# MrTornado24/IDE-3D

Hardware: AMD Instinct MI355X
Metric: 512x512 RGB+seg frames/s @96 depth samples (whole job) (higher is better)
Workload: dtype f32 (3x3 convs + MLPs: fp32 operands as 3 bf16 pieces, 6 products, f32 accumulate); 1 GPU; BASELINE config 2: random-init ide3d-ffhq-64-512, G.mapping + G.synthesis (64 render -> 512, 96 samples, RGB + 19-class seg) + uint8 frames, batch 4 seeds per GPU; global_batch=4, parallelism=dp1, conv_arithmetic=bf16x6, conv_arithmetic_is_library_default=True

## Files before the change

### ide-3d_amd/csrc/raymarch.hip

```cpp
#include "common.h"
#include "triplane_tap.h"
#include "raymarch_ray.h"

namespace ide3d {

typedef float f32x4 __attribute__((ext_vector_type(4)));

template <int C, int HID>
struct RmCfg {
    static constexpr int CPL = C / 16;
    static constexpr int NF = C / 4;
    static constexpr int MT1 = HID / 16;
    static constexpr int MT2 = 2;
    static constexpr int A1 = MT1 * CPL * 64 * 4;
    static constexpr int A2 = MT2 * MT1 * 64 * 4;
    static constexpr int B0 = MT1 * 16;
    static constexpr int B1 = MT2 * 16;
    static constexpr int MLP = A1 + A2 + B0 + B1;
};

template <int HID>
__device__ __forceinline__ void stage_out_fp32(float* __restrict__ a2, const float* __restrict__ w1, int nout) {
    constexpr int MT1 = HID / 16;
    for (int i = threadIdx.x; i < 2 * MT1 * 64 * 4; i += blockDim.x) {
// ... 58 lines not shown
        split_pair3(v[2 * e], v[2 * e + 1], pk);
        out[0][e] = pk[0]; out[1][e] = pk[1]; out[2][e] = pk[2];
    }
}
__device__ __forceinline__ f32x4 mfma6(const u32x4 (&a)[3], const u32x4 (&b)[3], f32x4 acc) {
#pragma unroll
    for (int sum = 2; sum >= 0; --sum)
#pragma unroll
        for (int qa = 0; qa <= sum; ++qa)
            acc = __builtin_amdgcn_mfma_f32_16x16x32_bf16(__builtin_bit_cast(bf16x8, a[qa]), __builtin_bit_cast(bf16x8, b[sum - qa]), acc, 0, 0, 0);
    return acc;
}

template <int C, int HID>
__device__ __forceinline__ void stage_split_layer1(u32x4* __restrict__ a1, const float* __restrict__ w0) {
    using K = RmSplit<C, HID>;
    for (int i = threadIdx.x; i < K::MT1 * 64; i += blockDim.x) {
        const int lane = i & 63, mt = i >> 6, g = lane >> 4, row = 16 * mt + (lane & 15);
        float v[8];
#pragma unroll
        for (int k = 0; k < 8; ++k) v[k] = w0[row * C + 16 * (k / 4) + 4 * g + k % 4];
        u32x4 pc[3];
        split8(v, pc);
#pragma unroll
        for (int q = 0; q < 3; ++q) a1[(mt * 3 + q) * 64 + lane] = pc[q];
    }
}
template <int HID>
__device__ __forceinline__ void stage_split_biases(float* __restrict__ sb, const float* __restrict__ b0, const float* __restrict__ b1, int nout) {
    for (int i = threadIdx.x; i < HID; i += blockDim.x) sb[i] = b0[i];
    for (int i = threadIdx.x; i < 32; i += blockDim.x) sb[HID + i] = (i < nout) ? b1[i] : 0.f;
}

template <int C, int HID>
__device__ void stage_mlp_split(unsigned char* __restrict__ sm, const float* __restrict__ w0, const float* __restrict__ b0,
                                const float* __restrict__ w1, const float* __restrict__ b1, int nout) {
    using K = RmSplit<C, HID>;
    u32x4* a1 = reinterpret_cast<u32x4*>(sm);
    u32x4* a2 = a1 + K::A1;
    stage_split_layer1<C, HID>(a1, w0);
    for (int i = threadIdx.x; i < 2 * K::KH * 64; i += blockDim.x) {
        const int lane = i & 63, kh = (i >> 6) % K::KH, m2 = i / (64 * K::KH), g = lane >> 4, row = 16 * m2 + (lane & 15);
        float v[8];
#pragma unroll
        for (int k = 0; k < 8; ++k) v[k] = (row < nout) ? w1[row * HID + 16 * (2 * kh + k / 4) + 4 * g + k % 4] : 0.f;
        u32x4 pc[3];
        split8(v, pc);
#pragma unroll
        for (int q = 0; q < 3; ++q) a2[((m2 * K::KH + kh) * 3 + q) * 64 + lane] = pc[q];
    }
    stage_split_biases<HID>(reinterpret_cast<float*>(a2 + K::A2), b0, b1, nout);
}

template <int C, int HID, int A2U = RmSplit<C, HID>::A2>
__device__ __forceinline__ void mlp_hidden_split(const unsigned char* __restrict__ sm, const float (&f)[C / 4], f32x4 (&h)[HID / 16]) {
    using K = RmSplit<C, HID>;
    const int lane = lane_id(), g = lane >> 4;
    const u32x4* a1 = reinterpret_cast<const u32x4*>(sm);
    const f32x4* sb0 = reinterpret_cast<const f32x4*>(sm + (K::A1 + A2U) * 16);
    u32x4 fb[3];
    split8(f, fb);
#pragma unroll
    for (int mt = 0; mt < K::MT1; ++mt) {
        const u32x4 a[3] = {a1[(mt * 3 + 0) * 64 + lane], a1[(mt * 3 + 1) * 64 + lane], a1[(mt * 3 + 2) * 64 + lane]};
        h[mt] = mfma6(a, fb, sb0[mt * 4 + g]);
    }
#pragma unroll
    for (int mt = 0; mt < K::MT1; ++mt)
#pragma unroll
        for (int r = 0; r < 4; ++r) h[mt][r] = softplus_fast(h[mt][r]);
}

template <int C, int HID>
__device__ __forceinline__ void mlp_tile_split(const unsigned char* __restrict__ sm, const float (&f)[C / 4], f32x4 (&out)[2]) {
    using K = RmSplit<C, HID>;
    const int lane = lane_id(), g = lane >> 4;
    const u32x4* a2 = reinterpret_cast<const u32x4*>(sm) + K::A1;
    const f32x4* sb1 = reinterpret_cast<const f32x4*>(sm + (K::A1 + K::A2) * 16) + K::MT1 * 4;
    f32x4 h[K::MT1];
    mlp_hidden_split<C, HID>(sm, f, h);
    u32x4 hb[K::KH][3];
#pragma unroll
    for (int kh = 0; kh < K::KH; ++kh) {
        const float v[8] = {h[2 * kh][0], h[2 * kh][1], h[2 * kh][2], h[2 * kh][3], h[2 * kh + 1][0], h[2 * kh + 1][1], h[2 * kh + 1][2], h[2 * kh + 1][3]};
        split8(v, hb[kh]);
    }
#pragma unroll
    for (int m2 = 0; m2 < 2; ++m2) {
        f32x4 acc = sb1[m2 * 4 + g];
#pragma unroll
        for (int kh = 0; kh < K::KH; ++kh) {
            const int o = ((m2 * K::KH + kh) * 3) * 64 + lane;
            const u32x4 a[3] = {a2[o], a2[o + 64], a2[o + 128]};
            acc = mfma6(a, hb[kh], acc);
        }
        out[m2] = acc;
    }
}

template <int HID>
__device__ __forceinline__ float sigma_row0(const float* __restrict__ s_row, const f32x4 (&h)[HID / 16]) {
    const int g = lane_id() >> 4;
    float acc = 0.f;
#pragma unroll
    for (int mt = 0; mt < HID / 16; ++mt) {
        const f32x4 w = *reinterpret_cast<const f32x4*>(s_row + 16 * mt + 4 * g);
#pragma unroll
        for (int r = 0; r < 4; ++r) acc += w[r] * h[mt][r];
    }
    acc += __shfl_xor(acc, 16);
    acc += __shfl_xor(acc, 32);
    return acc + s_row[HID];
}

template <int C, int HID>
__device__ __forceinline__ float mlp_sigma_split(const unsigned char* __restrict__ sm, const float* __restrict__ s_row, const float (&f)[C / 4]) {
    f32x4 h[HID / 16];
    mlp_hidden_split<C, HID>(sm, f, h);
    return sigma_row0<HID>(s_row, h);
}

__device__ __forceinline__ int gather_sample(int lane) { return lane >> 2; }
__device__ __forceinline__ int gather_block(int lane) { return lane & 3; }

template <int NF>
__device__ __forceinline__ void to_matrix_lanes(float (&f)[NF]) {
    const int lane = lane_id();
    const int src = (((lane & 15) << 2) | (lane >> 4)) << 2;
#pragma unroll
    for (int i = 0; i < NF; ++i) f[i] = __int_as_float(__builtin_amdgcn_ds_bpermute(src, __float_as_int(f[i])));
}

template <int C> struct TapBuf { float4 v[C / 16][3][4]; };

typedef const __attribute__((address_space(1))) char* GlobalBytes;
template <class T>
__device__ __forceinline__ GlobalBytes uniform_ptr(const T* p) {
    const unsigned long long v = reinterpret_cast<unsigned long long>(p);
    const unsigned lo = __builtin_amdgcn_readfirstlane((unsigned)v), hi = __builtin_amdgcn_readfirstlane((unsigned)(v >> 32));
    return reinterpret_cast<GlobalBytes>(((unsigned long long)hi << 32) | lo);
}

__device__ __forceinline__ float4 ld4_at(GlobalBytes base, unsigned byte_off, unsigned imm) {
    typedef float v4f __attribute__((ext_vector_type(4)));
    typedef const __attribute__((address_space(1))) v4f* GlobalF4;
    const v4f v = *reinterpret_cast<GlobalF4>(base + (size_t)byte_off + imm);
    return make_float4(v[0], v[1], v[2], v[3]);
}

template <int C>
__device__ __forceinline__ void issue_taps(GlobalBytes pbc, const TapAddr (&t)[3], int g, TapBuf<C>& b, unsigned lane_extra = 0) {
    constexpr int CPL = C / 16;
    const unsigned lane_b = 16u * (unsigned)g + lane_extra;
#pragma unroll
    for (int ci = 0; ci < CPL; ++ci) {
#pragma unroll
        for (int pl = 0; pl < 3; ++pl) {
            const unsigned imm = (unsigned)(pl * C + 16 * ci) * 4u;
            b.v[ci][pl][0] = ld4_at(pbc, (unsigned)t[pl].o00 * 4u + lane_b, imm); b.v[ci][pl][1] = ld4_at(pbc, (unsigned)t[pl].o01 * 4u + lane_b, imm);
            b.v[ci][pl][2] = ld4_at(pbc, (unsigned)t[pl].o10 * 4u + lane_b, imm); b.v[ci][pl][3] = ld4_at(pbc, (unsigned)t[pl].o11 * 4u + lane_b, imm);
        }
    }
}

template <int C>
__device__ __forceinline__ void blend_taps(TapBuf<C>& b, const TapAddr (&t)[3], float (&f)[C / 4]) {
    constexpr int CPL = C / 16;
#pragma unroll
    for (int ci = 0; ci < CPL; ++ci)
#pragma unroll
        for (int pl = 0; pl < 3; ++pl)
#pragma unroll
            for (int k = 0; k < 4; ++k) asm volatile("" : "+v"(b.v[ci][pl][k].x), "+v"(b.v[ci][pl][k].y), "+v"(b.v[ci][pl][k].z), "+v"(b.v[ci][pl][k].w));
#pragma unroll
    for (int ci = 0; ci < CPL; ++ci) {
        float4 a[3];
#pragma unroll
        for (int pl = 0; pl < 3; ++pl) {
            float4 acc = make_float4(0.f, 0.f, 0.f, 0.f);
            acc = f4_fma(b.v[ci][pl][0], t[pl].w00, acc);
            acc = f4_fma(b.v[ci][pl][1], t[pl].w01, acc);
            acc = f4_fma(b.v[ci][pl][2], t[pl].w10, acc);
            acc = f4_fma(b.v[ci][pl][3], t[pl].w11, acc);
            a[pl] = acc;
        }
        f[4 * ci + 0] = (a[0].x + a[1].x) + a[2].x;
        f[4 * ci + 1] = (a[0].y + a[1].y) + a[2].y;
        f[4 * ci + 2] = (a[0].z + a[1].z) + a[2].z;
        f[4 * ci + 3] = (a[0].w + a[1].w) + a[2].w;
    }
}

template <int C>
__device__ __forceinline__ void gather_features(const float* __restrict__ pb, const TapAddr (&t)[3], int g, float (&f)[C / 4]) {
    TapBuf<C> b;
    issue_taps<C>(uniform_ptr(pb), t, g, b);
    blend_taps<C>(b, t, f);
}

template <int C, int HID>
__device__ __forceinline__ void mlp_hidden(const float* __restrict__ s, const float (&f)[C / 4], f32x4 (&h)[HID / 16]) {
    using K = RmCfg<C, HID>;
    const int lane = lane_id();
    const f32x4* a1 = reinterpret_cast<const f32x4*>(s);
    const f32x4* sb0 = reinterpret_cast<const f32x4*>(s + K::A1 + K::A2);
    const int g = lane >> 4;
#pragma unroll
    for (int mt = 0; mt < K::MT1; ++mt) h[mt] = sb0[mt * 4 + g];
#pragma unroll
    for (int ci = 0; ci < K::CPL; ++ci) {
        f32x4 w[K::MT1];
#pragma unroll
        for (int mt = 0; mt < K::MT1; ++mt) w[mt] = a1[(mt * K::CPL + ci) * 64 + lane];
#pragma unroll
        for (int e = 0; e < 4; ++e)
#pragma unroll
            for (int mt = 0; mt < K::MT1; ++mt)
                h[mt] = __builtin_amdgcn_mfma_f32_16x16x4f32(w[mt][e], f[4 * ci + e], h[mt], 0, 0, 0);
    }
#pragma unroll
    for (int mt = 0; mt < K::MT1; ++mt)
#pragma unroll
        for (int r = 0; r < 4; ++r) h[mt][r] = softplus_fast(h[mt][r]);
}

template <int C, int HID>
__device__ __forceinline__ void mlp_tile(const float* __restrict__ s, const float (&f)[C / 4], f32x4 (&out)[2]) {
    using K = RmCfg<C, HID>;
    const int lane = lane_id();
    const f32x4* a2 = reinterpret_cast<const f32x4*>(s + K::A1);
    const f32x4* sb1 = reinterpret_cast<const f32x4*>(s + K::A1 + K::A2 + K::B0);
    const int g = lane >> 4;
    f32x4 h[K::MT1];
    mlp_hidden<C, HID>(s, f, h);
#pragma unroll
    for (int mt = 0; mt < 2; ++mt) out[mt] = sb1[mt * 4 + g];
#pragma unroll
    for (int tq = 0; tq < K::MT1; ++tq) {
        const f32x4 w0 = a2[(0 * K::MT1 + tq) * 64 + lane];
        const f32x4 w1 = a2[(1 * K::MT1 + tq) * 64 + lane];
#pragma unroll
        for (int e = 0; e < 4; ++e) {
            out[0] = __builtin_amdgcn_mfma_f32_16x16x4f32(w0[e], h[tq][e], out[0], 0, 0, 0);
            out[1] = __builtin_amdgcn_mfma_f32_16x16x4f32(w1[e], h[tq][e], out[1], 0, 0, 0);
        }
    }
}

template <int C, int HID>
__device__ __forceinline__ float mlp_sigma(const float* __restrict__ s, const float* __restrict__ s_row, const float (&f)[C / 4]) {
    f32x4 h[HID / 16];
    mlp_hidden<C, HID>(s, f, h);
    return sigma_row0<HID>(s_row, h);
}

__device__ __forceinline__ float seg16_excl_prod(float v, float& total) {
    const int j = lane_id() & 15;
    float incl = v;
#pragma unroll
    for (int off = 1; off < 16; off <<= 1) {
        const float o = __shfl_up(incl, off, 16);
        if (j >= off) incl *= o;
    }
    total = __shfl(incl, 15, 16);
    const float prev = __shfl_up(incl, 1, 16);
    return j == 0 ? 1.0f : prev;
}

template <int C, int HID, bool SPLIT> struct MlpBytes { static constexpr int value = RmCfg<C, HID>::MLP * 4; };
template <int C, int HID> struct MlpBytes<C, HID, true> { static constexpr int value = RmSplit<C, HID>::BYTES; };

template <int C, int HID, bool SPLIT>
__device__ __forceinline__ void stage_branch(unsigned char* sm, const float* w0, const float* b0, const float* w1, const float* b1, int nout) {
    if constexpr (SPLIT) stage_mlp_split<C, HID>(sm, w0, b0, w1, b1, nout);
    else stage_mlp<C, HID>(reinterpret_cast<float*>(sm), w0, b0, w1, b1, nout);
}
template <int C, int HID, bool SPLIT>
__device__ __forceinline__ void mlp_branch(const unsigned char* sm, const float (&f)[C / 4], f32x4 (&out)[2]) {
    if constexpr (SPLIT) mlp_tile_split<C, HID>(sm, f, out);
    else mlp_tile<C, HID>(reinterpret_cast<const float*>(sm), f, out);
}

template <int C, int HID, bool SPLIT> struct RmRender {
    using K = RmCfg<C, HID>;
    static constexpr int W2_OFF = K::A1 * 4, B1_OFF = (K::A1 + K::A2 + K::B0) * 4, BYTES = K::MLP * 4;
    static constexpr int ROW = HID + 4;
};
template <int C, int HID> struct RmRender<C, HID, true> {
    using K = RmSplit<C, HID>;
    static constexpr int W2 = 2 * K::MT1 * 64;
    static constexpr int W2_OFF = K::A1 * 16, B1_OFF = (K::A1 + W2) * 16 + HID * 4, BYTES = (K::A1 + W2) * 16 + K::BIAS * 4;
    static constexpr int ROW = HID + 4;
};

template <int C, int HID, bool SPLIT>
__device__ __forceinline__ void stage_render_branch(unsigned char* sm, const float* w0, const float* b0, const float* w1, const float* b1, int nout) {
    if constexpr (SPLIT) {
        using R = RmRender<C, HID, true>;
        stage_split_layer1<C, HID>(reinterpret_cast<u32x4*>(sm), w0);
        stage_out_fp32<HID>(reinterpret_cast<float*>(sm + R::W2_OFF), w1, nout);
        stage_split_biases<HID>(reinterpret_cast<float*>(sm + R::W2_OFF + R::W2 * 16), b0, b1, nout);
    } else {
        stage_mlp<C, HID>(reinterpret_cast<float*>(sm), w0, b0, w1, b1, nout);
    }
}
template <int C, int HID, bool SPLIT>
__device__ __forceinline__ void hidden_branch(const unsigned char* sm, const float (&f)[C / 4], f32x4 (&h)[HID / 16]) {
    if constexpr (SPLIT) mlp_hidden_split<C, HID, RmRender<C, HID, true>::W2>(sm, f, h);
    else mlp_hidden<C, HID>(reinterpret_cast<const float*>(sm), f, h);
}

template <int CTRL>
__device__ __forceinline__ float dpp_add(float v) {
    return v + __int_as_float(__builtin_amdgcn_update_dpp(0, __float_as_int(v), CTRL, 0xf, 0xf, false));
}
__device__ __forceinline__ float row16_sum(float v) {
    v = dpp_add<0xB1>(v); v = dpp_add<0x4E>(v); v = dpp_add<0x141>(v); v = dpp_add<0x140>(v);
    return v;
}

template <int C, int HID, bool SPLIT>
__device__ __forceinline__ void heads_per_ray(const unsigned char* sm, const float (&acc)[HID / 4], float wsum, float (&out)[2]) {
    using R = RmRender<C, HID, SPLIT>;
    constexpr int MT1 = HID / 16;
    const int lane = lane_id();
    const f32x4* w2 = reinterpret_cast<const f32x4*>(sm + R::W2_OFF);
    const float* sb1 = reinterpret_cast<const float*>(sm + R::B1_OFF);
#pragma unroll
    for (int m2 = 0; m2 < 2; ++m2) {
        float a = 0.f;
#pragma unroll
        for (int mt = 0; mt < MT1; ++mt) {
            const f32x4 w = w2[(m2 * MT1 + mt) * 64 + lane];
#pragma unroll
            for (int r = 0; r < 4; ++r) a = fmaf(w[r], acc[4 * mt + r], a);
        }
        a += __shfl_xor(a, 16);
        a += __shfl_xor(a, 32);
        out[m2] = fmaf(sb1[16 * m2 + (lane & 15)], wsum, a);
    }
}

template <bool SPLIT> struct RmWaves { static constexpr int value = SPLIT ? 8 : 4; };
template <bool SPLIT> __device__ __forceinline__ void rm_claim_half_simd() { if constexpr (SPLIT) asm volatile("" ::: "v255"); }

template <int C, int HID, bool SPLIT>
__global__ void __launch_bounds__(64 * RmWaves<SPLIT>::value, 2)
render_rays_kernel(ide3d_render_params p, int64_t rays_per_block) {
    using K = RmCfg<C, HID>;
    constexpr int NW = RmWaves<SPLIT>::value;
    rm_claim_half_simd<SPLIT>();
    extern __shared__ __attribute__((aligned(16))) float lds[];
    using R = RmRender<C, HID, SPLIT>;
    constexpr int NA = HID / 4;
    unsigned char* s_geo = reinterpret_cast<unsigned char*>(lds);
    unsigned char* s_tex = s_geo + R::BYTES;
    float* const s_row = reinterpret_cast<float*>(s_tex + R::BYTES);
    stage_render_branch<C, HID, SPLIT>(s_geo, p.geo_w0, p.geo_b0, p.geo_w1, p.geo_b1, 1 + p.seg_ch);
    stage_render_branch<C, HID, SPLIT>(s_tex, p.tex_w0, p.tex_b0, p.tex_w1, p.tex_b1, p.feat_ch);
    for (int i = threadIdx.x; i <= HID; i += blockDim.x) s_row[i] = (i < HID) ? p.geo_w1[i] : p.geo_b1[0];
    __syncthreads();

    const int lane = lane_id(), wid = __builtin_amdgcn_readfirstlane(threadIdx.x >> 6);
    const int g = lane >> 4, j = lane & 15, gl = gather_block(lane);
    const int64_t total_rays = (int64_t)p.n * p.rays_per_img;
    const int blk = xcd_remap(blockIdx.x, gridDim.x);
    const int64_t ray_begin = (int64_t)blk * rays_per_block;
    int64_t ray_end = ray_begin + rays_per_block;
    if (ray_end > total_rays) ray_end = total_rays;
    const int S = p.steps;
    const int nch = p.feat_ch + p.seg_ch;
    const int sH = (int)p.tex_stride[2], sW = (int)p.tex_stride[3];
    const float zstep = (S > 1) ? (p.z_lin[1] - p.z_lin[0]) : 0.f;

    auto tile_depth = [&](int64_t ray, int s0, float& zl, float& jl) {
        const int sl = min(s0 + gather_sample(lane), S - 1);
        zl = p.z_lin[sl];
        jl = p.jitter ? p.jitter[ray * S + sl] : 0.5f;
    };
    auto tile_taps = [&](int n, int r, float zl, float jl, TapAddr (&t)[3]) {
        float wx, wy, wz;
        ray_world_point(p, n, r, zl, jl, zstep, wx, wy, wz);
        t[0] = make_tap_addr(wx, wy, p.W, p.H, sH, sW);
        t[1] = make_tap_addr(wy, wz, p.W, p.H, sH, sW);
        t[2] = make_tap_addr(wx, wz, p.W, p.H, sH, sW);
    };

    int64_t ray = ray_begin + wid;
    int n = __builtin_amdgcn_readfirstlane((int)(ray / p.rays_per_img));
    int r = __builtin_amdgcn_readfirstlane((int)(ray - (int64_t)n * p.rays_per_img));
    int s0 = 0;
    bool have = ray < ray_end;
    TapAddr t[3];
    TapBuf<C> buf;
    if (have) {
        float zl, jl;
        tile_depth(ray, 0, zl, jl);
        tile_taps(n, r, zl, jl, t);
        issue_taps<C>(uniform_ptr(p.geo_planes + n * p.geo_stride[0]), t, gl, buf);
    }
    float acc_t[NA], acc_g[NA];
#pragma unroll
    for (int i = 0; i < NA; ++i) { acc_t[i] = 0.f; acc_g[i] = 0.f; }
    float carry = 1.0f, wsum = 0.f, dsum = 0.f;

    while (have) {
        int s0n = s0 + 16, nn = n, rn = r;
        int64_t rayn = ray;
        if (s0n >= S) {
            s0n = 0; rayn = ray + NW; rn = r + NW;
            while (rn >= p.rays_per_img) { rn -= (int)p.rays_per_img; ++nn; }
        }
        const bool haven = rayn < ray_end;
        const int64_t rayp = haven ? rayn : ray;
        const int np = haven ? nn : n, rp = haven ? rn : r, s0p = haven ? s0n : s0;
        const int s = s0 + j;
        const bool live = s < S;
        const int sc = live ? s : S - 1;
        float z = p.z_lin[sc];
        float znext = (sc + 1 < S) ? p.z_lin[sc + 1] : 0.f;
        if (p.jitter) {
            const float* jit = p.jitter + ray * S;
            z = __fadd_rn(z, __fmul_rn(__fsub_rn(jit[sc], 0.5f), zstep));
            if (sc + 1 < S) znext = __fadd_rn(znext, __fmul_rn(__fsub_rn(jit[sc + 1], 0.5f), zstep));
        }
        const float noise = p.sigma_noise ? p.sigma_noise[ray * S + sc] : 0.f;
        float zln, jln;
        tile_depth(rayp, s0p, zln, jln);

        float fg[K::NF], ft[K::NF];
        f32x4 hg[K::MT1], ht[K::MT1];
        blend_taps<C>(buf, t, fg);
        to_matrix_lanes(fg);
        issue_taps<C>(uniform_ptr(p.tex_planes + n * p.tex_stride[0]), t, gl, buf);
        hidden_branch<C, HID, SPLIT>(s_geo, fg, hg);

        float sigma = sigma_row0<HID>(s_row, hg);
        sigma += noise;
        const float dens = p.clamp_mode == 0 ? softplus_fast(sigma) : fmaxf(sigma, 0.f);
        float dnorm;
        {
            const float dx = p.rays_d_cam[r * 3 + 0], dy = p.rays_d_cam[r * 3 + 1], dz = p.rays_d_cam[r * 3 + 2];
            dnorm = sqrtf(dx * dx + dy * dy + dz * dz);
        }
        const float delta = (sc + 1 < S) ? (znext - z) * dnorm : 1e10f;
        const float alpha = live ? 1.0f - __expf(-delta * dens) : 0.f;
        const float fac = live ? (1.0f - alpha + 1e-10f) : 1.0f;
        float tot;
        const float excl = seg16_excl_prod(fac, tot);
        const float w = alpha * (carry * excl);
        carry *= tot;
        wsum += w; dsum += w * z;
#pragma unroll
        for (int mt = 0; mt < K::MT1; ++mt)
#pragma unroll
            for (int rr = 0; rr < 4; ++rr) acc_g[mt * 4 + rr] += w * hg[mt][rr];

        blend_taps<C>(buf, t, ft);
        to_matrix_lanes(ft);
        tile_taps(np, rp, zln, jln, t);
        issue_taps<C>(uniform_ptr(p.geo_planes + np * p.geo_stride[0]), t, gl, buf);
        hidden_branch<C, HID, SPLIT>(s_tex, ft, ht);
#pragma unroll
        for (int mt = 0; mt < K::MT1; ++mt)
#pragma unroll
            for (int rr = 0; rr < 4; ++rr) acc_t[mt * 4 + rr] += w * ht[mt][rr];

        if (s0n == 0) {
            wsum = row16_sum(wsum); dsum = row16_sum(dsum);
#pragma unroll
            for (int i = 0; i < NA; ++i) { acc_g[i] = row16_sum(acc_g[i]); acc_t[i] = row16_sum(acc_t[i]); }
            float o_t[2], o_g[2];
            heads_per_ray<C, HID, SPLIT>(s_tex, acc_t, wsum, o_t);
            heads_per_ray<C, HID, SPLIT>(s_geo, acc_g, wsum, o_g);
            {
                const float bg = p.white_back ? (1.0f - wsum) : 0.f;
                float* of = p.out_feat + (int64_t)n * nch * p.rays_per_img + r;
                const int idx = j + 16 * (g & 1);
                const float v = (g & 2) ? ((g & 1) ? o_g[1] : o_g[0]) : ((g & 1) ? o_t[1] : o_t[0]);
                if (g < 2) {
                    if (idx < p.feat_ch) of[(int64_t)idx * p.rays_per_img] = v + bg;
                } else {
                    if (idx >= 1 && idx <= p.seg_ch) of[(int64_t)(p.feat_ch + idx - 1) * p.rays_per_img] = v + bg;
                }
                if (lane == 0) {
                    if (p.out_depth) p.out_depth[ray] = dsum + ((p.max_depth != 0.f) ? (1.0f - wsum) * p.max_depth : 0.f);
                    if (p.out_wsum) p.out_wsum[ray] = wsum;
                }
            }
#pragma unroll
            for (int i = 0; i < NA; ++i) { acc_t[i] = 0.f; acc_g[i] = 0.f; }
            carry = 1.0f; wsum = 0.f; dsum = 0.f;
        }
        ray = rayn; n = nn; r = rn; s0 = s0n; have = haven;
    }
    if constexpr (SPLIT) __syncthreads();
}

struct PointsFromMemory {
    const float* pts;
    __device__ __forceinline__ void get(int64_t row, int64_t , float& x, float& y, float& z) const {
        x = pts[row * 3 + 0]; y = pts[row * 3 + 1]; z = pts[row * 3 + 2];
    }
};

struct PointsFromLattice {
    ide3d_lattice lat;
    int64_t first;
    __device__ __forceinline__ void get(int64_t , int64_t idx, float& x, float& y, float& z) const {
        const int64_t i = first + idx;
        const float fn = (float)lat.n, fi = (float)i;
        const float q = __fdiv_rn(fi, fn);
        const int64_t r2 = (i >> 32) == 0 ? (int64_t)((unsigned)i % (unsigned)lat.n) : i % lat.n;
        const float s2 = (float)r2, s1 = fmodf(q, fn), s0 = fmodf(__fdiv_rn(q, fn), fn);
        x = __fmul_rn(__fadd_rn(__fmul_rn(s0, lat.voxel_size), lat.corner[2]), lat.scale);
        y = __fmul_rn(__fadd_rn(__fmul_rn(s1, lat.voxel_size), lat.corner[1]), lat.scale);
        z = __fmul_rn(__fadd_rn(__fmul_rn(s2, lat.voxel_size), lat.corner[0]), lat.scale);
    }
};

template <class Src>
__global__ void lattice_points_kernel(Src src, int64_t count, float* __restrict__ out) {
    for (int64_t i = (int64_t)blockIdx.x * blockDim.x + threadIdx.x; i < count; i += (int64_t)gridDim.x * blockDim.x) {
        float x, y, z;
        src.get(i, i, x, y, z);
        out[i * 3 + 0] = x; out[i * 3 + 1] = y; out[i * 3 + 2] = z;
    }
}

template <int C, int HID, class Src, bool SPLIT>
__global__ void __launch_bounds__(64 * RmWaves<SPLIT>::value, 2)
sample_voxel_kernel(ide3d_render_params p, const Src src, int64_t m, float* __restrict__ out, int64_t tiles_per_block) {
    using K = RmCfg<C, HID>;
    constexpr int NW = RmWaves<SPLIT>::value;
    rm_claim_half_simd<SPLIT>();
    extern __shared__ __attribute__((aligned(16))) float lds[];
    constexpr int MB = MlpBytes<C, HID, SPLIT>::value;
    unsigned char* s_geo = reinterpret_cast<unsigned char*>(lds);
    unsigned char* s_tex = s_geo + MB;
    float* s_stage = reinterpret_cast<float*>(s_geo + 2 * MB);
    stage_branch<C, HID, SPLIT>(s_geo, p.geo_w0, p.geo_b0, p.geo_w1, p.geo_b1, 1 + p.seg_ch);
    stage_branch<C, HID, SPLIT>(s_tex, p.tex_w0, p.tex_b0, p.tex_w1, p.tex_b1, p.feat_ch);
    __syncthreads();
    const int lane = lane_id(), wid = __builtin_amdgcn_readfirstlane(threadIdx.x >> 6);
    const int g = lane >> 4, j = lane & 15, gl = gather_block(lane);
    const int width = p.feat_ch + p.seg_ch + 1;
    const int sH = (int)p.tex_stride[2], sW = (int)p.tex_stride[3];
// ... 115 lines not shown
        src.get(rc, rc - (e - m), wx, wy, wz);
        tl[0] = make_tap_addr(wx, wy, p.W, p.H, sH, sW);
        tl[1] = make_tap_addr(wy, wz, p.W, p.H, sH, sW);
        tl[2] = make_tap_addr(wx, wz, p.W, p.H, sH, sW);
    };
    auto tile_taps = [&](const TapAddr (&tl)[3], int dnl, int k, TapAddr (&t)[3], int& dn) {
        const int src_b = (16 * k + gather_sample(lane)) << 2;
#pragma unroll
        for (int pl = 0; pl < 3; ++pl) {
            t[pl].o00 = __builtin_amdgcn_ds_bpermute(src_b, tl[pl].o00); t[pl].o01 = __builtin_amdgcn_ds_bpermute(src_b, tl[pl].o01);
            t[pl].o10 = __builtin_amdgcn_ds_bpermute(src_b, tl[pl].o10); t[pl].o11 = __builtin_amdgcn_ds_bpermute(src_b, tl[pl].o11);
            t[pl].w00 = __int_as_float(__builtin_amdgcn_ds_bpermute(src_b, __float_as_int(tl[pl].w00)));
            t[pl].w01 = __int_as_float(__builtin_amdgcn_ds_bpermute(src_b, __float_as_int(tl[pl].w01)));
            t[pl].w10 = __int_as_float(__builtin_amdgcn_ds_bpermute(src_b, __float_as_int(tl[pl].w10)));
            t[pl].w11 = __int_as_float(__builtin_amdgcn_ds_bpermute(src_b, __float_as_int(tl[pl].w11)));
        }
        dn = __builtin_amdgcn_ds_bpermute(src_b, dnl);
    };

    int64_t st = super_begin + wid;
    if (st < super_end) {
    TapAddr tl[3], t[3];
    TapBuf<C> buf;
    int dnl, dn;
    super_taps(st, tl, dnl);
    tile_taps(tl, dnl, 0, t, dn);
    issue_taps<C>(uniform_ptr(p.geo_planes + n0 * p.geo_stride[0]), t, gl, buf, (unsigned)dn * geo_img_b);
    while (st < super_end) {
        const int64_t stn = st + NW;
        const int64_t stp = stn < super_end ? stn : st;
#pragma unroll
        for (int k = 0; k < 4; ++k) {
            const int64_t row = st * 64 + 16 * k + j;
            float fg[K::NF];
            blend_taps<C>(buf, t, fg);
            to_matrix_lanes(fg);
            if (k == 3) super_taps(stp, tl, dnl);
            tile_taps(tl, dnl, (k + 1) & 3, t, dn);
            issue_taps<C>(uniform_ptr(p.geo_planes + n0 * p.geo_stride[0]), t, gl, buf, (unsigned)dn * geo_img_b);
            float sig;
            if constexpr (SPLIT) sig = mlp_sigma_split<C, HID>(s_geo, s_row, fg);
            else sig = mlp_sigma<C, HID>(reinterpret_cast<const float*>(s_geo), s_row, fg);
            if (g == 0 && row < rows) out_sigma[row] = sig;
        }
        st = stn;
    }
    }
    if constexpr (SPLIT) __syncthreads();
}

template <int C, int HID, bool SPLIT = false>
static int launch_render(const ide3d_render_params& p, hipStream_t st) {
    using R = RmRender<C, HID, SPLIT>;
    const size_t lds_bytes = (size_t)2 * R::BYTES + (size_t)R::ROW * sizeof(float);
    const int64_t total_rays = (int64_t)p.n * p.rays_per_img;
    constexpr int NW = RmWaves<SPLIT>::value;
    int64_t nblk = kNumCU * 8 / NW;
    int64_t rpb = cdiv64(cdiv64(total_rays, nblk), NW) * NW;
    if (rpb < NW) rpb = NW;
    nblk = cdiv64(total_rays, rpb);
    auto kern = render_rays_kernel<C, HID, SPLIT>;
    (void)hipFuncSetAttribute(reinterpret_cast<const void*>(kern), hipFuncAttributeMaxDynamicSharedMemorySize, (int)lds_bytes);
    if constexpr (SPLIT) IDE3D_EXCL_LAUNCH(kern, dim3((unsigned)nblk), 64 * NW, lds_bytes, st, p, rpb);
    else hipLaunchKernelGGL(kern, dim3((unsigned)nblk), dim3(64 * NW), lds_bytes, st, p, rpb);
    IDE3D_CHECK_LAUNCH("render_rays");
    return IDE3D_OK;
}

template <int C, int HID, class Src, bool SPLIT = false>
static int launch_voxel(const ide3d_render_params& p, const Src& src, int64_t m, float* out, float* out_sigma,
                        int sigma_only, hipStream_t st) {
    constexpr int NW = RmWaves<SPLIT>::value;
    {
        const int64_t rows_per_tile = sigma_only ? 64 : 16;
        const int64_t max_dn = (p.n > 1) ? ((rows_per_tile - 1) / (m > 0 ? m : 1) + 1 < p.n - 1 ? (rows_per_tile - 1) / (m > 0 ? m : 1) + 1 : p.n - 1) : 0;
        const int64_t img = p.geo_stride[0] > p.tex_stride[0] ? p.geo_stride[0] : p.tex_stride[0];
        if ((max_dn * img + img) * 4 >= 0xffffffffLL) { set_error("sample_voxel: too few points per image for planes this large"); return IDE3D_ENOKERNEL; }
    }
    if (sigma_only) {
        const size_t lds_bytes = (size_t)MlpBytes<C, HID, SPLIT>::value + (size_t)(HID + 4) * sizeof(float);
        const int64_t nsuper = cdiv64((int64_t)p.n * m, 64);
        int64_t nblk = kNumCU * 8 / NW;
        int64_t spb = cdiv64(cdiv64(nsuper, nblk), NW) * NW;
        if (spb < NW) spb = NW;
        nblk = cdiv64(nsuper, spb);
        auto kern = density_kernel<C, HID, Src, SPLIT>;
        (void)hipFuncSetAttribute(reinterpret_cast<const void*>(kern), hipFuncAttributeMaxDynamicSharedMemorySize, (int)lds_bytes);
        if constexpr (SPLIT) IDE3D_EXCL_LAUNCH(kern, dim3((unsigned)nblk), 64 * NW, lds_bytes, st, p, src, m, out_sigma, spb);
        else hipLaunchKernelGGL(kern, dim3((unsigned)nblk), dim3(64 * NW), lds_bytes, st, p, src, m, out_sigma, spb);
        IDE3D_CHECK_LAUNCH("sample_voxel (densities)");
        return IDE3D_OK;
    }
    const int width = p.feat_ch + p.seg_ch + 1;
    const size_t lds_bytes = (size_t)2 * MlpBytes<C, HID, SPLIT>::value + (size_t)NW * 16 * width * sizeof(float);
    const int64_t ntiles = cdiv64((int64_t)p.n * m, 16);
    int64_t nblk = kNumCU * 8 / NW;
    int64_t tpb = cdiv64(cdiv64(ntiles, nblk), NW) * NW;
    if (tpb < NW) tpb = NW;
    nblk = cdiv64(ntiles, tpb);
    auto kern = sample_voxel_kernel<C, HID, Src, SPLIT>;
    (void)hipFuncSetAttribute(reinterpret_cast<const void*>(kern), hipFuncAttributeMaxDynamicSharedMemorySize, (int)lds_bytes);
    if constexpr (SPLIT) IDE3D_EXCL_LAUNCH(kern, dim3((unsigned)nblk), 64 * NW, lds_bytes, st, p, src, m, out, tpb);
    else hipLaunchKernelGGL(kern, dim3((unsigned)nblk), dim3(64 * NW), lds_bytes, st, p, src, m, out, tpb);
    IDE3D_CHECK_LAUNCH("sample_voxel");
    return IDE3D_OK;
}

}

static bool mlp_split_selected() { return ide3d_get_conv_arithmetic() != 1; }

extern "C" int ide3d_render_rays(const ide3d_render_params* pp, void* stream) {
// ... 86 lines not shown
```

### ide-3d_amd/csrc/raymarch_ray.h

```cpp
#pragma once
#include "common.h"
#include "triplane_tap.h"

namespace ide3d {

__device__ __forceinline__ float softplus_fast(float x) {
    const float e = __builtin_amdgcn_exp2f(-1.44269504088896340736f * fabsf(x));
    return fmaf(0.69314718055994530942f, __builtin_amdgcn_logf(1.0f + e), fmaxf(x, 0.f));
}

__device__ __forceinline__ float ray_sample_depth(const ide3d_render_params& p, int64_t ray, int s, float zstep) {
    const float z = p.z_lin[s];
    return p.jitter ? __fadd_rn(z, __fmul_rn(__fsub_rn(p.jitter[ray * p.steps + s], 0.5f), zstep)) : z;
}

__device__ __forceinline__ void ray_camera_point(const ide3d_render_params& p, int r, float zl, float jl, float zstep,
                                                 float& px, float& py, float& pz) {
    const float dx = p.rays_d_cam[r * 3 + 0], dy = p.rays_d_cam[r * 3 + 1], dz = p.rays_d_cam[r * 3 + 2];
    px = __fmul_rn(dx, zl); py = __fmul_rn(dy, zl); pz = __fmul_rn(dz, zl);
    if (p.jitter) {
        const float off = __fmul_rn(__fsub_rn(jl, 0.5f), zstep);
        px = __fadd_rn(px, __fmul_rn(off, dx));
        py = __fadd_rn(py, __fmul_rn(off, dy));
        pz = __fadd_rn(pz, __fmul_rn(off, dz));
    }
}

__device__ __forceinline__ void ray_world_point(const ide3d_render_params& p, int n, int r, float zl, float jl, float zstep,
                                                float& wx, float& wy, float& wz) {
    const float dx = p.rays_d_cam[r * 3 + 0], dy = p.rays_d_cam[r * 3 + 1], dz = p.rays_d_cam[r * 3 + 2];
    const float* M = p.cam2world + n * 16;
    float px = __fmul_rn(dx, zl), py = __fmul_rn(dy, zl), pz = __fmul_rn(dz, zl);
    if (p.jitter) {
        const float off = __fmul_rn(__fsub_rn(jl, 0.5f), zstep);
        px = __fadd_rn(px, __fmul_rn(off, dx));
        py = __fadd_rn(py, __fmul_rn(off, dy));
        pz = __fadd_rn(pz, __fmul_rn(off, dz));
    }
    wx = fmaf(M[0], px, fmaf(M[1], py, fmaf(M[2], pz, M[3])));
    wy = fmaf(M[4], px, fmaf(M[5], py, fmaf(M[6], pz, M[7])));
    wz = fmaf(M[8], px, fmaf(M[9], py, fmaf(M[10], pz, M[11])));
}

__device__ __forceinline__ void triplane_taps(float wx, float wy, float wz, int W, int H, Tap2 (&t)[3]) {
    t[0] = make_tap(wx, wy, W, H);
    t[1] = make_tap(wy, wz, W, H);
    t[2] = make_tap(wx, wz, W, H);
}


static inline int check_render_params(const ide3d_render_params& p, const char* who, bool need_rays) {
    IDE3D_CHECK_ARG(p.tex_planes && p.geo_planes, "%s: null tri-plane pointer", who);
    IDE3D_CHECK_ARG(p.geo_w0 && p.geo_b0 && p.geo_w1 && p.geo_b1 && p.tex_w0 && p.tex_b0 && p.tex_w1 && p.tex_b1,
                    "%s: null MLP weight pointer", who);
    IDE3D_CHECK_ARG(p.n > 0 && p.C > 0 && p.H > 0 && p.W > 0, "%s: bad tri-plane shape", who);
    IDE3D_CHECK_ARG(p.feat_ch >= 1 && p.feat_ch <= 32 && p.seg_ch >= 0 && p.seg_ch <= 31,
                    "%s: feat_ch <= 32 and seg_ch <= 31 required", who);
    if (need_rays) {
        IDE3D_CHECK_ARG(p.rays_d_cam && p.z_lin && p.cam2world && p.out_feat, "%s: null ray / output pointer", who);
        IDE3D_CHECK_ARG(p.rays_per_img > 0 && p.steps > 0, "%s: bad ray shape", who);
        IDE3D_CHECK_ARG(p.clamp_mode == 0 || p.clamp_mode == 1, "%s: Need to choose clamp mode", who);
    }
    return IDE3D_OK;
}

static inline bool planes_fast(const ide3d_render_params& p) {
    auto ok = [&](const float* base, const int64_t* s) {
        return s[1] == 1 && (s[0] % 4 == 0) && (s[2] % 4 == 0) && (s[3] % 4 == 0) &&
               ((reinterpret_cast<uintptr_t>(base) & 15) == 0);
    };
    return ok(p.tex_planes, p.tex_stride) && ok(p.geo_planes, p.geo_stride) &&
           p.tex_stride[2] == p.geo_stride[2] && p.tex_stride[3] == p.geo_stride[3] &&
           (p.tex_stride[2] * p.H + p.tex_stride[3] * p.W + 3 * p.C) * 4 < 0x7fffffffLL;
}

}
```

Measured before the change: 938.3 frames/s.

## Restructure render ray loop: LDS depth table, per-ray constants, DPP tap sharing

Reworks the fused render kernel's per-tile loop. The depth table now lives in LDS. Jitter and noise rows are loaded once per tile and distributed with bpermute, and ray direction and camera matrix are loaded once per ray through constant-address-space scalar loads. Each lane computes tap addresses for only one plane, and the three planes are exchanged via DPP quad broadcasts. Softplus uses med3 instead of max, and ray bookkeeping moves to a Tile struct with 32-bit ray indices plus new LDS and ray-count limit checks. This aims to cut redundant global loads and VALU address math in the raymarch inner loop, at the cost of extra cross-lane ops and an LDS-size constraint on the step count.

Result: no change. 946.7 frames/s, median of 6 (+0.9%).

```diff
diff --git a/ide-3d_amd/csrc/raymarch.hip b/ide-3d_amd/csrc/raymarch.hip
--- a/ide-3d_amd/csrc/raymarch.hip
+++ b/ide-3d_amd/csrc/raymarch.hip
@@ -134,8 +134,8 @@
     stage_split_biases<HID>(reinterpret_cast<float*>(a2 + K::A2), b0, b1, nout);
 }
 
-template <int C, int HID, int A2U = RmSplit<C, HID>::A2>
-__device__ __forceinline__ void mlp_hidden_split(const unsigned char* __restrict__ sm, const float (&f)[C / 4], f32x4 (&h)[HID / 16]) {
+template <int C, int HID, int A2U = RmSplit<C, HID>::A2, bool MED3 = false>
+__device__ __forceinline__ void mlp_hidden_split(const unsigned char* __restrict__ sm, const float (&f)[C / 4], f32x4 (&h)[HID / 16], float pos_inf = 0.f) {
     using K = RmSplit<C, HID>;
     const int lane = lane_id(), g = lane >> 4;
     const u32x4* a1 = reinterpret_cast<const u32x4*>(sm);
@@ -150,7 +150,7 @@
 #pragma unroll
     for (int mt = 0; mt < K::MT1; ++mt)
 #pragma unroll
-        for (int r = 0; r < 4; ++r) h[mt][r] = softplus_fast(h[mt][r]);
+        for (int r = 0; r < 4; ++r) h[mt][r] = MED3 ? softplus_fast_med3(h[mt][r], pos_inf) : softplus_fast(h[mt][r]);
 }
 
 template <int C, int HID>
@@ -223,11 +223,27 @@
     return reinterpret_cast<GlobalBytes>(((unsigned long long)hi << 32) | lo);
 }
 
+typedef const __attribute__((address_space(4))) float* ConstFloats;
+__device__ __forceinline__ ConstFloats const_floats(const float* p) {
+    return reinterpret_cast<ConstFloats>(reinterpret_cast<unsigned long long>(p));
+}
+
 __device__ __forceinline__ float4 ld4_at(GlobalBytes base, unsigned byte_off, unsigned imm) {
     typedef float v4f __attribute__((ext_vector_type(4)));
     typedef const __attribute__((address_space(1))) v4f* GlobalF4;
     const v4f v = *reinterpret_cast<GlobalF4>(base + (size_t)byte_off + imm);
     return make_float4(v[0], v[1], v[2], v[3]);
+}
+
+template <int Q>
+__device__ __forceinline__ void quad_taps(const TapAddr& m, TapAddr& t) {
+    constexpr int CTRL = Q * 0x55;
+    t.o00 = __builtin_amdgcn_update_dpp(0, m.o00, CTRL, 0xf, 0xf, false); t.o01 = __builtin_amdgcn_update_dpp(0, m.o01, CTRL, 0xf, 0xf, false);
+    t.o10 = __builtin_amdgcn_update_dpp(0, m.o10, CTRL, 0xf, 0xf, false); t.o11 = __builtin_amdgcn_update_dpp(0, m.o11, CTRL, 0xf, 0xf, false);
+    t.w00 = __int_as_float(__builtin_amdgcn_update_dpp(0, __float_as_int(m.w00), CTRL, 0xf, 0xf, false));
+    t.w01 = __int_as_float(__builtin_amdgcn_update_dpp(0, __float_as_int(m.w01), CTRL, 0xf, 0xf, false));
+    t.w10 = __int_as_float(__builtin_amdgcn_update_dpp(0, __float_as_int(m.w10), CTRL, 0xf, 0xf, false));
+    t.w11 = __int_as_float(__builtin_amdgcn_update_dpp(0, __float_as_int(m.w11), CTRL, 0xf, 0xf, false));
 }
 
 template <int C>
@@ -280,8 +296,8 @@
     blend_taps<C>(b, t, f);
 }
 
-template <int C, int HID>
-__device__ __forceinline__ void mlp_hidden(const float* __restrict__ s, const float (&f)[C / 4], f32x4 (&h)[HID / 16]) {
+template <int C, int HID, bool MED3 = false>
+__device__ __forceinline__ void mlp_hidden(const float* __restrict__ s, const float (&f)[C / 4], f32x4 (&h)[HID / 16], float pos_inf = 0.f) {
     using K = RmCfg<C, HID>;
     const int lane = lane_id();
     const f32x4* a1 = reinterpret_cast<const f32x4*>(s);
@@ -303,7 +319,7 @@
 #pragma unroll
     for (int mt = 0; mt < K::MT1; ++mt)
 #pragma unroll
-        for (int r = 0; r < 4; ++r) h[mt][r] = softplus_fast(h[mt][r]);
+        for (int r = 0; r < 4; ++r) h[mt][r] = MED3 ? softplus_fast_med3(h[mt][r], pos_inf) : softplus_fast(h[mt][r]);
 }
 
 template <int C, int HID>
@@ -387,9 +403,9 @@
     }
 }
 template <int C, int HID, bool SPLIT>
-__device__ __forceinline__ void hidden_branch(const unsigned char* sm, const float (&f)[C / 4], f32x4 (&h)[HID / 16]) {
-    if constexpr (SPLIT) mlp_hidden_split<C, HID, RmRender<C, HID, true>::W2>(sm, f, h);
-    else mlp_hidden<C, HID>(reinterpret_cast<const float*>(sm), f, h);
+__device__ __forceinline__ void hidden_branch(const unsigned char* sm, const float (&f)[C / 4], f32x4 (&h)[HID / 16], float pos_inf) {
+    if constexpr (SPLIT) mlp_hidden_split<C, HID, RmRender<C, HID, true>::W2, true>(sm, f, h, pos_inf);
+    else mlp_hidden<C, HID, true>(reinterpret_cast<const float*>(sm), f, h, pos_inf);
 }
 
 template <int CTRL>
@@ -438,9 +454,11 @@
     unsigned char* s_geo = reinterpret_cast<unsigned char*>(lds);
     unsigned char* s_tex = s_geo + R::BYTES;
     float* const s_row = reinterpret_cast<float*>(s_tex + R::BYTES);
+    float* const s_z = s_row + R::ROW;
     stage_render_branch<C, HID, SPLIT>(s_geo, p.geo_w0, p.geo_b0, p.geo_w1, p.geo_b1, 1 + p.seg_ch);
     stage_render_branch<C, HID, SPLIT>(s_tex, p.tex_w0, p.tex_b0, p.tex_w1, p.tex_b1, p.feat_ch);
     for (int i = threadIdx.x; i <= HID; i += blockDim.x) s_row[i] = (i < HID) ? p.geo_w1[i] : p.geo_b1[0];
+    for (int i = threadIdx.x; i < p.steps; i += blockDim.x) s_z[i] = p.z_lin[i];
     __syncthreads();
 
     const int lane = lane_id(), wid = __builtin_amdgcn_readfirstlane(threadIdx.x >> 6);
@@ -450,81 +468,102 @@
     const int64_t ray_begin = (int64_t)blk * rays_per_block;
     int64_t ray_end = ray_begin + rays_per_block;
     if (ray_end > total_rays) ray_end = total_rays;
+    const int nr = __builtin_amdgcn_readfirstlane((int)(ray_end - ray_begin));
     const int S = p.steps;
     const int nch = p.feat_ch + p.seg_ch;
     const int sH = (int)p.tex_stride[2], sW = (int)p.tex_stride[3];
     const float zstep = (S > 1) ? (p.z_lin[1] - p.z_lin[0]) : 0.f;
-
-    auto tile_depth = [&](int64_t ray, int s0, float& zl, float& jl) {
-        const int sl = min(s0 + gather_sample(lane), S - 1);
-        zl = p.z_lin[sl];
-        jl = p.jitter ? p.jitter[ray * S + sl] : 0.5f;
+    const bool jittered = p.jitter != nullptr;
+    const float pos_inf = opaque_pos_inf();
+
+    struct Tile { int kr, n, r, s0; };
+    auto next_tile = [&](const Tile& c, bool& ok) {
+        Tile d = c;
+        d.s0 += 16;
+        if (d.s0 >= S) {
+            d.s0 = 0; d.kr += NW; d.r += NW;
+            while (d.r >= p.rays_per_img) { d.r -= p.rays_per_img; ++d.n; }
+        }
+        ok = d.kr < nr;
+        return ok ? d : c;
     };
-    auto tile_taps = [&](int n, int r, float zl, float jl, TapAddr (&t)[3]) {
+    auto ray_consts = [&](const Tile& c, RayConsts& rc) {
+        const ConstFloats d = const_floats(p.rays_d_cam) + c.r * 3, M = const_floats(p.cam2world) + c.n * 16;
+        rc.dx = d[0]; rc.dy = d[1]; rc.dz = d[2];
+#pragma unroll
+        for (int i = 0; i < 12; ++i) rc.m[i] = M[i];
+    };
+    auto tile_loads = [&](const Tile& c, float& jrow, float& nrow) {
+        const int sl = min(c.s0 + lane, S - 1);
+        const int64_t base = (ray_begin + c.kr) * S;
+        const float* jp = p.jitter ? p.jitter + base : p.z_lin;
+        const float* np = p.sigma_noise ? p.sigma_noise + base : p.z_lin;
+        jrow = jp[sl]; nrow = np[sl];
+    };
+    auto tile_taps = [&](const Tile& c, const RayConsts& rc, float jrow, TapAddr (&t)[3]) {
+        const int sl = min(c.s0 + gather_sample(lane), S - 1);
+        const float zl = s_z[sl];
+        const float jl = __int_as_float(__builtin_amdgcn_ds_bpermute((sl - c.s0) << 2, __float_as_int(jrow)));
         float wx, wy, wz;
-        ray_world_point(p, n, r, zl, jl, zstep, wx, wy, wz);
-        t[0] = make_tap_addr(wx, wy, p.W, p.H, sH, sW);
-        t[1] = make_tap_addr(wy, wz, p.W, p.H, sH, sW);
-        t[2] = make_tap_addr(wx, wz, p.W, p.H, sH, sW);
+        ray_world_point_from(jittered, rc, zl, jl, zstep, wx, wy, wz);
+        const TapAddr m = make_tap_addr(gl == 1 ? wy : wx, gl == 0 ? wy : wz, p.W, p.H, sH, sW);
+        quad_taps<0>(m, t[0]); quad_taps<1>(m, t[1]); quad_taps<2>(m, t[2]);
     };
 
-    int64_t ray = ray_begin + wid;
-    int n = __builtin_amdgcn_readfirstlane((int)(ray / p.rays_per_img));
-    int r = __builtin_amdgcn_readfirstlane((int)(ray - (int64_t)n * p.rays_per_img));
-    int s0 = 0;
-    bool have = ray < ray_end;
+    Tile cur;
+    {
+        const int64_t ray = ray_begin + wid;
+        cur.kr = wid;
+        cur.n = __builtin_amdgcn_readfirstlane((int)(ray / p.rays_per_img));
+        cur.r = __builtin_amdgcn_readfirstlane((int)(ray - (int64_t)cur.n * p.rays_per_img));
+        cur.s0 = 0;
+    }
+    bool have = cur.kr < nr;
+    if (have) {
+    RayConsts rc;
+    float nj, nn;
     TapAddr t[3];
     TapBuf<C> buf;
-    if (have) {
-        float zl, jl;
-        tile_depth(ray, 0, zl, jl);
-        tile_taps(n, r, zl, jl, t);
-        issue_taps<C>(uniform_ptr(p.geo_planes + n * p.geo_stride[0]), t, gl, buf);
-    }
+    ray_consts(cur, rc);
+    tile_loads(cur, nj, nn);
+    float dnorm = sqrtf(rc.dx * rc.dx + rc.dy * rc.dy + rc.dz * rc.dz);
+    tile_taps(cur, rc, nj, t);
+    issue_taps<C>(uniform_ptr(p.geo_planes + cur.n * p.geo_stride[0]), t, gl, buf);
     float acc_t[NA], acc_g[NA];
 #pragma unroll
     for (int i = 0; i < NA; ++i) { acc_t[i] = 0.f; acc_g[i] = 0.f; }
     float carry = 1.0f, wsum = 0.f, dsum = 0.f;
 
     while (have) {
-        int s0n = s0 + 16, nn = n, rn = r;
-        int64_t rayn = ray;
-        if (s0n >= S) {
-            s0n = 0; rayn = ray + NW; rn = r + NW;
-            while (rn >= p.rays_per_img) { rn -= (int)p.rays_per_img; ++nn; }
-        }
-        const bool haven = rayn < ray_end;
-        const int64_t rayp = haven ? rayn : ray;
-        const int np = haven ? nn : n, rp = haven ? rn : r, s0p = haven ? s0n : s0;
-        const int s = s0 + j;
+        bool more;
+        const Tile nxt = next_tile(cur, more);
+        const bool ray_done = cur.s0 + 16 >= S;
+        const float cj = nj, cn = nn;
+        tile_loads(nxt, nj, nn);
+        const int s = cur.s0 + j;
         const bool live = s < S;
         const int sc = live ? s : S - 1;
-        float z = p.z_lin[sc];
-        float znext = (sc + 1 < S) ? p.z_lin[sc + 1] : 0.f;
-        if (p.jitter) {
-            const float* jit = p.jitter + ray * S;
-            z = __fadd_rn(z, __fmul_rn(__fsub_rn(jit[sc], 0.5f), zstep));
-            if (sc + 1 < S) znext = __fadd_rn(znext, __fmul_rn(__fsub_rn(jit[sc + 1], 0.5f), zstep));
+        const int sc1 = (sc + 1 < S) ? sc + 1 : sc;
+        float z = s_z[sc];
+        float znext = (sc + 1 < S) ? s_z[sc1] : 0.f;
+        if (jittered) {
+            const float jz = __int_as_float(__builtin_amdgcn_ds_bpermute((sc - cur.s0) << 2, __float_as_int(cj)));
+            const float jz1 = __int_as_float(__builtin_amdgcn_ds_bpermute((sc1 - cur.s0) << 2, __float_as_int(cj)));
+            z = __fadd_rn(z, __fmul_rn(__fsub_rn(jz, 0.5f), zstep));
+            if (sc + 1 < S) znext = __fadd_rn(znext, __fmul_rn(__fsub_rn(jz1, 0.5f), zstep));
         }
-        const float noise = p.sigma_noise ? p.sigma_noise[ray * S + sc] : 0.f;
-        float zln, jln;
-        tile_depth(rayp, s0p, zln, jln);
+        const float noise = p.sigma_noise ? __int_as_float(__builtin_amdgcn_ds_bpermute((sc - cur.s0) << 2, __float_as_int(cn))) : 0.f;
 
         float fg[K::NF], ft[K::NF];
         f32x4 hg[K::MT1], ht[K::MT1];
         blend_taps<C>(buf, t, fg);
         to_matrix_lanes(fg);
-        issue_taps<C>(uniform_ptr(p.tex_planes + n * p.tex_stride[0]), t, gl, buf);
-        hidden_branch<C, HID, SPLIT>(s_geo, fg, hg);
+        issue_taps<C>(uniform_ptr(p.tex_planes + cur.n * p.tex_stride[0]), t, gl, buf);
+        hidden_branch<C, HID, SPLIT>(s_geo, fg, hg, pos_inf);
 
         float sigma = sigma_row0<HID>(s_row, hg);
         sigma += noise;
-        const float dens = p.clamp_mode == 0 ? softplus_fast(sigma) : fmaxf(sigma, 0.f);
-        float dnorm;
-        {
-            const float dx = p.rays_d_cam[r * 3 + 0], dy = p.rays_d_cam[r * 3 + 1], dz = p.rays_d_cam[r * 3 + 2];
-            dnorm = sqrtf(dx * dx + dy * dy + dz * dz);
-        }
+        const float dens = p.clamp_mode == 0 ? softplus_fast_med3(sigma, pos_inf) : fmaxf(sigma, 0.f);
         const float delta = (sc + 1 < S) ? (znext - z) * dnorm : 1e10f;
         const float alpha = live ? 1.0f - __expf(-delta * dens) : 0.f;
         const float fac = live ? (1.0f - alpha + 1e-10f) : 1.0f;
@@ -538,17 +577,19 @@
 #pragma unroll
             for (int rr = 0; rr < 4; ++rr) acc_g[mt * 4 + rr] += w * hg[mt][rr];
 
+        if (ray_done) ray_consts(nxt, rc);
         blend_taps<C>(buf, t, ft);
         to_matrix_lanes(ft);
-        tile_taps(np, rp, zln, jln, t);
-        issue_taps<C>(uniform_ptr(p.geo_planes + np * p.geo_stride[0]), t, gl, buf);
-        hidden_branch<C, HID, SPLIT>(s_tex, ft, ht);
+        tile_taps(nxt, rc, nj, t);
+        issue_taps<C>(uniform_ptr(p.geo_planes + nxt.n * p.geo_stride[0]), t, gl, buf);
+        if (ray_done) dnorm = sqrtf(rc.dx * rc.dx + rc.dy * rc.dy + rc.dz * rc.dz);
+        hidden_branch<C, HID, SPLIT>(s_tex, ft, ht, pos_inf);
 #pragma unroll
         for (int mt = 0; mt < K::MT1; ++mt)
 #pragma unroll
             for (int rr = 0; rr < 4; ++rr) acc_t[mt * 4 + rr] += w * ht[mt][rr];
 
-        if (s0n == 0) {
+        if (ray_done) {
             wsum = row16_sum(wsum); dsum = row16_sum(dsum);
 #pragma unroll
             for (int i = 0; i < NA; ++i) { acc_g[i] = row16_sum(acc_g[i]); acc_t[i] = row16_sum(acc_t[i]); }
@@ -557,7 +598,7 @@
             heads_per_ray<C, HID, SPLIT>(s_geo, acc_g, wsum, o_g);
             {
                 const float bg = p.white_back ? (1.0f - wsum) : 0.f;
-                float* of = p.out_feat + (int64_t)n * nch * p.rays_per_img + r;
+                float* of = p.out_feat + (int64_t)cur.n * nch * p.rays_per_img + cur.r;
                 const int idx = j + 16 * (g & 1);
                 const float v = (g & 2) ? ((g & 1) ? o_g[1] : o_g[0]) : ((g & 1) ? o_t[1] : o_t[0]);
                 if (g < 2) {
@@ -566,6 +607,7 @@
                     if (idx >= 1 && idx <= p.seg_ch) of[(int64_t)(p.feat_ch + idx - 1) * p.rays_per_img] = v + bg;
                 }
                 if (lane == 0) {
+                    const int64_t ray = ray_begin + cur.kr;
                     if (p.out_depth) p.out_depth[ray] = dsum + ((p.max_depth != 0.f) ? (1.0f - wsum) * p.max_depth : 0.f);
                     if (p.out_wsum) p.out_wsum[ray] = wsum;
                 }
@@ -574,7 +616,8 @@
             for (int i = 0; i < NA; ++i) { acc_t[i] = 0.f; acc_g[i] = 0.f; }
             carry = 1.0f; wsum = 0.f; dsum = 0.f;
         }
-        ray = rayn; n = nn; r = rn; s0 = s0n; have = haven;
+        cur = nxt; have = more;
+    }
     }
     if constexpr (SPLIT) __syncthreads();
 }
@@ -796,12 +839,14 @@
 template <int C, int HID, bool SPLIT = false>
 static int launch_render(const ide3d_render_params& p, hipStream_t st) {
     using R = RmRender<C, HID, SPLIT>;
-    const size_t lds_bytes = (size_t)2 * R::BYTES + (size_t)R::ROW * sizeof(float);
+    const size_t lds_bytes = (size_t)2 * R::BYTES + (size_t)R::ROW * sizeof(float) + (((size_t)p.steps + 3) / 4) * 16;
+    if (lds_bytes > (size_t)160 * 1024) { set_error("render_rays: %d steps do not fit the depth table in LDS", (int)p.steps); return IDE3D_ENOKERNEL; }
     const int64_t total_rays = (int64_t)p.n * p.rays_per_img;
     constexpr int NW = RmWaves<SPLIT>::value;
     int64_t nblk = kNumCU * 8 / NW;
     int64_t rpb = cdiv64(cdiv64(total_rays, nblk), NW) * NW;
     if (rpb < NW) rpb = NW;
+    if (rpb > 0x7fffffffLL - NW) { set_error("render_rays: too many rays per workgroup"); return IDE3D_ENOKERNEL; }
     nblk = cdiv64(total_rays, rpb);
     auto kern = render_rays_kernel<C, HID, SPLIT>;
     (void)hipFuncSetAttribute(reinterpret_cast<const void*>(kern), hipFuncAttributeMaxDynamicSharedMemorySize, (int)lds_bytes);
diff --git a/ide-3d_amd/csrc/raymarch_ray.h b/ide-3d_amd/csrc/raymarch_ray.h
--- a/ide-3d_amd/csrc/raymarch_ray.h
+++ b/ide-3d_amd/csrc/raymarch_ray.h
@@ -7,6 +7,16 @@
 __device__ __forceinline__ float softplus_fast(float x) {
     const float e = __builtin_amdgcn_exp2f(-1.44269504088896340736f * fabsf(x));
     return fmaf(0.69314718055994530942f, __builtin_amdgcn_logf(1.0f + e), fmaxf(x, 0.f));
+}
+
+__device__ __forceinline__ float opaque_pos_inf() {
+    float v = __builtin_inff();
+    asm volatile("" : "+s"(v));
+    return v;
+}
+__device__ __forceinline__ float softplus_fast_med3(float x, float pos_inf) {
+    const float e = __builtin_amdgcn_exp2f(-1.44269504088896340736f * fabsf(x));
+    return fmaf(0.69314718055994530942f, __builtin_amdgcn_logf(1.0f + e), __builtin_amdgcn_fmed3f(x, 0.f, pos_inf));
 }
 
 __device__ __forceinline__ float ray_sample_depth(const ide3d_render_params& p, int64_t ray, int s, float zstep) {
@@ -42,6 +52,25 @@
     wz = fmaf(M[8], px, fmaf(M[9], py, fmaf(M[10], pz, M[11])));
 }
 
+struct RayConsts {
+    float dx, dy, dz;
+    float m[12];
+};
+
+__device__ __forceinline__ void ray_world_point_from(bool jittered, const RayConsts& c, float zl, float jl, float zstep,
+                                                     float& wx, float& wy, float& wz) {
+    float px = __fmul_rn(c.dx, zl), py = __fmul_rn(c.dy, zl), pz = __fmul_rn(c.dz, zl);
+    if (jittered) {
+        const float off = __fmul_rn(__fsub_rn(jl, 0.5f), zstep);
+        px = __fadd_rn(px, __fmul_rn(off, c.dx));
+        py = __fadd_rn(py, __fmul_rn(off, c.dy));
+        pz = __fadd_rn(pz, __fmul_rn(off, c.dz));
+    }
+    wx = fmaf(c.m[0], px, fmaf(c.m[1], py, fmaf(c.m[2], pz, c.m[3])));
+    wy = fmaf(c.m[4], px, fmaf(c.m[5], py, fmaf(c.m[6], pz, c.m[7])));
+    wz = fmaf(c.m[8], px, fmaf(c.m[9], py, fmaf(c.m[10], pz, c.m[11])));
+}
+
 __device__ __forceinline__ void triplane_taps(float wx, float wy, float wz, int W, int H, Tap2 (&t)[3]) {
     t[0] = make_tap(wx, wy, W, H);
     t[1] = make_tap(wy, wz, W, H);
```
